# openai/Video-Pre-Training

Hardware: AMD Instinct MI355X
Metric: frames/sec (fwd) [+ bc_step.ms_per_step], 2x policy, 128x128x3 seq=128 (higher is better)
Workload: dtype bf16; 1 GPU; foundation-model-2x policy forward (IMPALA CNN + 4-layer banded transformer + heads), batch=64 seq=128 uint8 128x128x3 frames per GPU, KV memory carried, random-init weights; global_batch=64, seq_len=128, parallelism=dp1 replicas (no collective in forward; BC step: gradient all-reduce)

## Files before the change

### include/vpt_hip.h

```cpp
#ifndef VPT_HIP_H
#define VPT_HIP_H
#include <stdint.h>

#ifdef __cplusplus
extern "C" {
#endif

const char* vpt_version(void);
#define VPT_HIP_ABI 5
int vpt_abi_version(void);
const char* vpt_operand_format(void);
const char* vpt_last_error(void);

long vpt_conv3x3_packed_elems(int Cout, int Cin);
long vpt_conv3x3_table_floats(int Cout);
long vpt_linear_packed_elems(int N, int K);
long vpt_conv_first_packed_elems(int Cout);
long vpt_conv3d_t5_packed_elems(int O);
int vpt_pack_conv_first(const float* weight, const float* bias, void* wfrag, int Cout, void* stream);
int vpt_pack_conv3d_t5(const float* weight, const float* bias, void* wfrag, float* bias_padded, int O, void* stream);
int vpt_chw_to_blocked(const float* src, float* dst, int64_t rows, int C, int H, int W, void* stream);

enum { VPT_WS_CONV3X3_WGRAD = 1, VPT_WS_CONV_BACKWARD_PREPARE = 2, VPT_WS_LINEAR_SPLITK = 3, VPT_WS_LAYERNORM_BACKWARD = 4, VPT_WS_COLUMN_SUM = 5,
       VPT_WS_ATTENTION_BACKWARD_DKV = 6, VPT_WS_ATTENTION_BACKWARD_DBND = 7, VPT_WS_FRAME_AFFINE_BACKWARD = 8, VPT_WS_CONV_FIRST_BACKWARD = 9,
// ... 47 lines not shown

int vpt_linear_forward(const void* A, const void* wpk, const float* bias, const float* res,
                       float* out_f32, void* out_bf16, int M, int N, int K,
                       int lda, int ldr, int ldc, int ldcb, int relu, int splitk, const void* mask, int ldm,
                       void* stream);
int vpt_linear_forward_tiled(const void* A, const void* wpk, const float* bias, const float* res,
                             float* out_f32, void* out_bf16, int M, int N, int K,
                             int lda, int ldr, int ldc, int ldcb, int relu, int splitk, const void* mask, int ldm,
                             int tiling, void* stream);

int vpt_linear_wgrad(const void* dy, const void* x, float* dw, int M, int N, int K, int ldy, int ldx, int ldw, int accumulate, void* stream);

int vpt_dense_fold_epilogue(const float* part, int splitk, const double* stats, int count, const float* sg, const float* sb, float* out,
                            int M, int N, void* stream);

int vpt_linear_splitk_epilogue(const float* part, int splitk, const float* bias, const float* res, float* out_f32, void* out_bf16,
                               int M, int N, int ldr, int ldc, int ldcb, int relu, const void* mask, int ldm, void* stream);

int vpt_layernorm_linear_forward(const float* x, const float* ln_gain, const float* ln_bias, int relu_in, float* ln_out_f32,
                                 const void* wpk, const float* bias, const float* res, float* out_f32, void* out_bf16,
                                 int M, int N, int K, int ldr, int ldc, int ldcb, int relu, void* stream);

int vpt_layernorm_forward(const float* x, const float* gain, const float* bias, float* out_f32, void* out_bf16,
                          int M, int D, int relu_in, void* stream);

int vpt_masked_attention_forward(const float* qkvr, const float* kmem, const float* vmem, const uint8_t* memvalid,
                                 const float* b_nd, void* out, int B, int t, int heads, int hid, int ld,
                                 int maxlen, int causal, void* stream);

int vpt_masked_attention_forward_episodes(const float* qkvr, const float* kmem, const float* vmem, const uint8_t* memvalid,
                                          const float* b_nd, void* out, const int32_t* qlo, int B, int t, int heads, int hid, int ld,
                                          int maxlen, void* stream);

int vpt_episode_bounds(const uint8_t* first, const uint8_t* state_mask, int32_t* qlo, uint8_t* mask_out, int B, int t, int maxlen, void* stream);

int vpt_kv_memory_update(const float* qkvr, const float* kmem, const float* vmem, float* kout, float* vout,
                         int B, int t, int hid, int ld, int maxlen, void* stream);

int vpt_masked_attention_step(const float* qkvr, const float* kmem, const float* vmem, const uint8_t* state_mask, const uint8_t* first,
                              const float* b_nd, void* out, float* kout, float* vout, uint8_t* mask_out,
                              int B, int heads, int hid, int ld, int maxlen, void* stream);

int vpt_masked_attention_step_inplace(const float* qkvr, float* kmem, float* vmem, uint8_t* state_mask, const uint8_t* first,
                                      const float* b_nd, void* out, int* done_counter, int B, int heads, int hid, int ld, int maxlen, void* stream);

int vpt_act_epilogue(const int64_t* action_buttons, const int64_t* action_camera, const float* logp_buttons, const float* logp_camera,
                     const float* logits, int ld, int value_col, float scale, float shift, int64_t* keep, uint8_t* nan_flag, uint64_t* rng_state,
                     int B, void* stream);

int vpt_log_softmax_forward(const float* logits, float* out, int M, int ld, int col0, int n, float temperature,
                            void* stream);

int vpt_action_head_forward(const float* logits, const uint8_t* mask, const float* noise, const uint64_t* rng_state, uint32_t rng_stream,
                            float* out, int64_t* action, float* action_logp, int M, int ld, int col0, int n, float temperature, void* stream);
int vpt_uniform_noise(const uint64_t* rng_state, uint32_t rng_stream, float* out, int M, int n, void* stream);

int vpt_adam_step(float* param, const float* grad, float* exp_avg, float* exp_avg_sq, uint64_t n, int step,
                  float lr, float beta1, float beta2, float eps, float weight_decay, float grad_scale, void* stream);

int vpt_adam_step_multi(const void* table, int ntensors, int64_t total_blocks, int step, float lr, float beta1, float beta2,
                        float eps, float weight_decay, float grad_scale, const int32_t* skip_flag, void* stream);

int vpt_grads_nonfinite_multi(const void* table, int ntensors, int64_t total_blocks, int32_t* flag, void* stream);

long vpt_grad_norm_workspace_bytes(int ntensors, int64_t total_blocks);
int vpt_grad_norm_multi(const void* table, int ntensors, int64_t total_blocks, float grad_scale, float max_norm, void* workspace,
// ... 133 lines not shown
```

### video-pre-training_amd/_native.py

```python
import ctypes
import os

_HERE = os.path.dirname(os.path.abspath(__file__))
_LIB_PATH = os.environ.get("VPT_HIP_LIB") or os.path.join(_HERE, "libvpt_hip.so")
_LIB_PATHS = {"bf16": _LIB_PATH, "fp16": os.path.join(_HERE, "libvpt_hip_f16.so")}
_libs = {}

ABI_VERSION = 5

_P = ctypes.c_void_p
_I = ctypes.c_int
_F = ctypes.c_float
_L = ctypes.c_long
_D = ctypes.c_double

SIGNATURES = {
    "vpt_conv_first_forward": [_P, _P, _P, _P, _P, _P, _I, _I, _I, _I, _P],
    "vpt_conv3d_t5_forward": [_P, _P, _P, _P, _P, _I, _I, _I, _I, _I, _P],
    "vpt_conv3d_t5_forward_indexed": [_P, _P, _P, _P, _P, _P, _P, _P, _I, _I, _I, _I, _I, _P],
    "vpt_conv3d_t5_backward": [_P, _P, _P, _P, _P, _P, _I, _I, _I, _I, _I, _P],
    "vpt_gather_rows": [_P, _P, _P, _L, _L, _I, _P],
    "vpt_idm_decode": [_P] * 9 + [_L, _I, _D, _D, _D, _I, _P],
    "vpt_pack_conv3x3": [_P, _P, _P, _P, _P, _P, _I, _I, _P],
    "vpt_pack_linear": [_P, _P, _I, _I, _I, _I, _I, _P],
# ... 37 lines not shown
    "vpt_frame_affine_backward": [_P, _P, _P, _P, _P, _P, _P, _P, _P, _P, _I, _I, _I, _I, _I, _P],
    "vpt_bc_nll_backward": [_P, _P, _P, _P, _P, _I, _I, _I, _I, _F, _P],
    "vpt_bc_loss": [_P, _P, _P, _P, _P, _P, _P, _P, _P, _I, _I, _I, _I, _F, _P],
    "vpt_idm_loss": [_P, _P, _P, _P, _P, _P, _P, _P, _P, _I, _I, _I, _I, _I, _I, _F, _P],
    "vpt_rl_loss": [_P] * 9 + [ctypes.c_int64] + [_P] * 7 + [_I, _I, _I, _I, _F, _F, _F, _F, _F, _F, _P],
    "vpt_ppg_aux_loss": [_P] * 5 + [ctypes.c_int64] + [_P] * 7 + [_I, _I, _I, _I, _F, _F, _F, _F, _P],
    "vpt_gae": [_P, _P, _P, _P, _P, _P, _P, _I, _I, _F, _F, _P],
    "vpt_rollout_record": [_P] * 6 + [ctypes.c_int64] * 4 + [_P] * 7 + [_I, _I, _I, ctypes.c_int64, _P],
    "vpt_rollout_reward": [_P] * 7 + [_I, _I, _I, _P],
    "vpt_full_attention_backward": [_P, _P, _P, _P, _I, _I, _I, _I, _I, _P],
    "vpt_heads_logprob_backward": [_P, _P, _P, _P, _P, _P, _P, _P, _I, _I, _I, _I, _F, _F, _P],
    "vpt_grouped_logprob_backward": [_P, _P, _P, _P, _P, _P, _P, _I, _I, _I, _I, _I, _I, _F, _F, _P],
    "vpt_layernorm_backward": [_P, _P, _P, _P, _P, _P, _P, _P, _I, _I, _I, _P],
    "vpt_gate_cast": [_P, _P, _P, _I, _I, _I, _I, _I, _P],
    "vpt_column_sum": [_P, _P, _P, _I, _I, _I, _P],
    "vpt_masked_attention_backward": [_P, _P, _P, _P, _P, _P, _P, _P, _P, _P, _I, _I, _I, _I, _I, _I, _P],
    "vpt_adam_step": [_P, _P, _P, _P, ctypes.c_uint64, _I, _F, _F, _F, _F, _F, _F, _P],
    "vpt_adam_step_multi": [_P, _I, _L, _I, _F, _F, _F, _F, _F, _F, _P, _P],
    "vpt_grads_nonfinite_multi": [_P, _I, _L, _P, _P],
    "vpt_grad_norm_workspace_bytes": [_I, ctypes.c_int64],
    "vpt_grad_norm_multi": [_P, _I, _L, _F, _F, _P, _P, _P, _P, _P],
    "vpt_adam_step_multi_clip": [_P, _I, _L, _I, _F, _F, _F, _F, _F, _F, _P, _P, _P],
    "vpt_grad_accumulate_multi": [_P, _I, _L, _P],
    "vpt_layernorm_linear_forward": [_P, _P, _P, _I, _P, _P, _P, _P, _P, _P, _I, _I, _I, _I, _I, _I, _I, _P],
    "vpt_masked_attention_step": [_P, _P, _P, _P, _P, _P, _P, _P, _P, _P, _I, _I, _I, _I, _I, _P],
    "vpt_masked_attention_step_inplace": [_P, _P, _P, _P, _P, _P, _P, _P, _I, _I, _I, _I, _I, _P],
    "vpt_act_epilogue": [_P, _P, _P, _P, _P, _I, _I, _F, _F, _P, _P, _P, _I, _P],
    "vpt_clip_frames": [_P, _I, _I, _I, _P, _P, _P, _I, _I, _P, _I, _I, _P],
    "vpt_augment_uniforms": [_P, _P, _L, ctypes.c_uint64, ctypes.c_uint32, _P],
    "vpt_augment_frames": [_P, _P, _P, _L, _I, _I, _P],
    "vpt_debug_poison_lds": [_P],
    "vpt_episode_bounds": [_P, _P, _P, _P, _I, _I, _I, _P],
    "vpt_masked_attention_forward_episodes": [_P, _P, _P, _P, _P, _P, _P, _I, _I, _I, _I, _I, _I, _P],
    "vpt_masked_attention_backward_episodes": [_P, _P, _P, _P, _P, _P, _P, _P, _P, _P, _P, _I, _I, _I, _I, _I, _I, _P],
}


class NativeLibraryError(RuntimeError):
    pass


def lib_path():
    return _LIB_PATH


def load(fmt: str = "bf16"):
    if fmt in _libs:
        return _libs[fmt]
    import torch
    path = _LIB_PATHS[fmt]
    if not os.path.exists(path):
        raise NativeLibraryError(
            f"{path} is missing: run `python __graft_entry__.py` (build()) first; there is no CPU fallback")
    lib = ctypes.CDLL(path)
    try:
        lib.vpt_abi_version.restype = ctypes.c_int
        abi = int(lib.vpt_abi_version())
    except AttributeError:
        abi = None
    if abi != ABI_VERSION:
        raise NativeLibraryError(f"{path} has C-ABI version {abi}, this package binds version {ABI_VERSION}: rebuild it (`python __graft_entry__.py`)")
    override = fmt == "bf16" and bool(os.environ.get("VPT_HIP_LIB"))
    for name, argtypes in SIGNATURES.items():
        try:
            fn = getattr(lib, name)
        except AttributeError:
# ... 32 lines not shown
```

### video-pre-training_amd/csrc/vpt_capi.hip

```cpp
#include "../../include/vpt_hip.h"
#include "vpt_kernels.h"
#include "vpt_common.h"
#include <stdio.h>
#include <math.h>

static thread_local char g_err[256] = "ok";

static int fail(int code, const char* what) {
  snprintf(g_err, sizeof(g_err), "%s (code %d, hip: %s)", what, code, hipGetErrorString(hipPeekAtLastError()));
  return code;
}
#define CHECK_LAUNCH(expr, name) do { int rc_ = (expr); if (rc_ != 0) return fail(rc_, name); return 0; } while (0)

__global__ __launch_bounds__(256) void vpt_poison_lds_kernel(int words, unsigned pattern) {
  extern __shared__ unsigned poison_lds_[];
  volatile unsigned* l = poison_lds_;
  for (int i = threadIdx.x; i < words; i += 256) l[i] = pattern;
  __syncthreads();
  for (int k = 0; k < 16; ++k) __builtin_amdgcn_s_sleep(127);
}

extern "C" {

const char* vpt_version(void) { return "vpt_hip 0.5 gfx950"; }
// ... 393 lines not shown
  a.A = nullptr; a.wpk = nullptr; a.bias = bias; a.res = res; a.out_f32 = out_f32; a.out_bf16 = (vpt_op16*)out_bf16;
  a.M = M; a.N = N; a.K = 0; a.lda = 0; a.ldr = ldr; a.ldc = ldc; a.ldcb = ldcb; a.relu = relu; a.splitk = splitk; a.atomic_out = 0;
  a.mask = (const vpt_op16*)mask; a.ldm = ldm;
  CHECK_LAUNCH(vpt_splitk_epilogue_launch(part, splitk, &a, (hipStream_t)stream), "vpt_linear_splitk_epilogue");
}

int vpt_layernorm_forward(const float* x, const float* gain, const float* bias, float* out_f32, void* out_bf16,
                          int M, int D, int relu_in, void* stream) {
  VptLayerNormArgs a = {};
  a.x = x; a.gain = gain; a.bias = bias; a.out_f32 = out_f32; a.out_bf16 = (vpt_op16*)out_bf16;
  a.M = M; a.D = D; a.relu_in = relu_in;
  CHECK_LAUNCH(vpt_layernorm_launch(&a, (hipStream_t)stream), "vpt_layernorm_forward");
}

int vpt_masked_attention_forward(const float* qkvr, const float* kmem, const float* vmem, const uint8_t* memvalid,
                                 const float* b_nd, void* out, int B, int t, int heads, int hid, int ld,
                                 int maxlen, int causal, void* stream) {
  VptAttnArgs a = {};
  a.qkvr = qkvr; a.kmem = kmem; a.vmem = vmem; a.memvalid = memvalid; a.b_nd = b_nd; a.out = (vpt_op16*)out;
  a.B = B; a.t = t; a.heads = heads; a.hid = hid; a.ld = ld; a.maxlen = maxlen; a.causal = causal;
  CHECK_LAUNCH(vpt_attn_launch(&a, (hipStream_t)stream), "vpt_masked_attention_forward");
}

int vpt_masked_attention_forward_episodes(const float* qkvr, const float* kmem, const float* vmem, const uint8_t* memvalid,
                                          const float* b_nd, void* out, const int32_t* qlo, int B, int t, int heads, int hid, int ld,
                                          int maxlen, void* stream) {
  if (!qlo) return fail(-1, "vpt_masked_attention_forward_episodes: qlo ([B*t] int32, vpt_episode_bounds) is required");
  VptAttnArgs a = {};
  a.qkvr = qkvr; a.kmem = kmem; a.vmem = vmem; a.memvalid = memvalid; a.b_nd = b_nd; a.out = (vpt_op16*)out; a.qlo = qlo;
  a.B = B; a.t = t; a.heads = heads; a.hid = hid; a.ld = ld; a.maxlen = maxlen; a.causal = 1;
  CHECK_LAUNCH(vpt_attn_launch(&a, (hipStream_t)stream), "vpt_masked_attention_forward_episodes");
}

int vpt_episode_bounds(const uint8_t* first, const uint8_t* state_mask, int32_t* qlo, uint8_t* mask_out, int B, int t, int maxlen, void* stream) {
  if (!first || B <= 0 || t < 1 || maxlen < 1) return fail(-1, "vpt_episode_bounds: first [B][t] with B, t, maxlen >= 1 is required");
  if (mask_out && !state_mask) return fail(-1, "vpt_episode_bounds: mask_out needs state_mask");
  if (mask_out && mask_out == state_mask) return fail(-1, "vpt_episode_bounds: mask_out must not alias state_mask");
  CHECK_LAUNCH(vpt_episode_bounds_launch(first, state_mask, qlo, mask_out, B, t, maxlen, (hipStream_t)stream), "vpt_episode_bounds");
}

int vpt_masked_attention_step(const float* qkvr, const float* kmem, const float* vmem, const uint8_t* state_mask, const uint8_t* first,
                              const float* b_nd, void* out, float* kout, float* vout, uint8_t* mask_out,
                              int B, int heads, int hid, int ld, int maxlen, void* stream) {
  VptAttnArgs a = {};
  a.qkvr = qkvr; a.kmem = kmem; a.vmem = vmem; a.memvalid = nullptr; a.b_nd = b_nd; a.out = (vpt_op16*)out;
  a.B = B; a.t = 1; a.heads = heads; a.hid = hid; a.ld = ld; a.maxlen = maxlen; a.causal = 1;
  CHECK_LAUNCH(vpt_attn_step_launch(&a, state_mask, first, mask_out, kout, vout, nullptr, (hipStream_t)stream), "vpt_masked_attention_step");
}

int vpt_masked_attention_step_inplace(const float* qkvr, float* kmem, float* vmem, uint8_t* state_mask, const uint8_t* first,
                                      const float* b_nd, void* out, int* done_counter, int B, int heads, int hid, int ld, int maxlen, void* stream) {
  if (!done_counter) return fail(-1, "vpt_masked_attention_step_inplace: done_counter ([B] ints, zero before the first launch) is required");
  VptAttnArgs a = {};
  a.qkvr = qkvr; a.kmem = kmem; a.vmem = vmem; a.memvalid = nullptr; a.b_nd = b_nd; a.out = (vpt_op16*)out;
  a.B = B; a.t = 1; a.heads = heads; a.hid = hid; a.ld = ld; a.maxlen = maxlen; a.causal = 1;
  CHECK_LAUNCH(vpt_attn_step_launch(&a, state_mask, first, state_mask, kmem, vmem, done_counter, (hipStream_t)stream), "vpt_masked_attention_step_inplace");
}

int vpt_act_epilogue(const int64_t* action_buttons, const int64_t* action_camera, const float* logp_buttons, const float* logp_camera,
                     const float* logits, int ld, int value_col, float scale, float shift, int64_t* keep, uint8_t* nan_flag, uint64_t* rng_state,
                     int B, void* stream) {
  CHECK_LAUNCH(vpt_act_epilogue_launch(action_buttons, action_camera, logp_buttons, logp_camera, logits, ld, value_col, scale, shift, keep, nan_flag,
                                       rng_state, B, (hipStream_t)stream), "vpt_act_epilogue");
}

int vpt_uniform_noise(const uint64_t* rng_state, uint32_t rng_stream, float* out, int M, int n, void* stream) {
// ... 355 lines not shown
```

### video-pre-training_amd/csrc/vpt_kernels.h

```cpp
#pragma once
#include <hip/hip_runtime.h>
#include <stdint.h>

#ifdef VPT_OPERAND_F16
typedef _Float16 vpt_op16;
#else
typedef __bf16 vpt_op16;
#endif

struct VptConv3x3Args {
  const vpt_op16* x;
  const vpt_op16* wpk;
  const float* edge_sa;
  const float* edge_sg;
  const double* stats_in;
  const vpt_op16* res;
  vpt_op16* y;
  double* stats_out;
  int frames, H, W, Cin, Cout, CoutPad, NT;
  double inv_count_in;
  int tiling;
  int ablate;
  long long* trace;
  const float* kk_frame;
// ... 124 lines not shown
  int ldm;
  const float* ln_x;
  const float* ln_gain;
  const float* ln_bias;
  float* ln_out_f32;
  int ln_relu_in;
};

struct VptGemmTnArgs {
  const vpt_op16* A;
  const vpt_op16* B;
  float* C;
  int M, N1, N2, lda, ldb, ldc, accumulate;
};

struct VptLayerNormArgs {
  const float* x;
  const float* gain;
  const float* bias;
  float* out_f32;
  vpt_op16* out_bf16;
  int M, D, relu_in;
};

struct VptAttnArgs {
  const float* qkvr;
  const float* kmem;
  const float* vmem;
  const uint8_t* memvalid;
  const float* b_nd;
  vpt_op16* out;
  int B, t, heads, hid, ld, maxlen, causal;
  const int32_t* qlo;
};

struct VptKvUpdateArgs {
  const float* qkvr;
  const float* kmem;
  const float* vmem;
  float* kout;
  float* vout;
  int B, t, hid, ld, maxlen;
};

struct VptLogSoftmaxArgs {
  const float* logits;
  float* out;
  int M, ld, col0, n;
  float temperature;
  const uint8_t* mask;
  const float* noise;
  const uint64_t* rng_state;
  uint32_t rng_stream;
  long* action;
  float* action_logp;
};

struct VptAffineBwdArgs {
  const vpt_op16* x;
  const vpt_op16* dy;
  const vpt_op16* dx_add;
  vpt_op16* dx;
  const float* gain;
  const double* stats_in;
  double* ab;
  float* dgain;
// ... 373 lines not shown
```

### video-pre-training_amd/csrc/vpt_transformer.hip

```cpp
#include "vpt_common.h"
#include "vpt_kernels.h"

__global__ __launch_bounds__(256) void vpt_layernorm_kernel(VptLayerNormArgs a) {
  const int lane = threadIdx.x & 63;
  const int row = blockIdx.x * 4 + (threadIdx.x >> 6);
  if (row >= a.M) return;
  const float* x = a.x + (size_t)row * a.D;
  const int n4 = a.D >> 2;
  float s = 0.f;
  for (int i = lane; i < n4; i += 64) {
    f32x4 v = *(const f32x4*)(x + 4 * i);
    if (a.relu_in) { v.x = fmaxf(v.x, 0.f); v.y = fmaxf(v.y, 0.f); v.z = fmaxf(v.z, 0.f); v.w = fmaxf(v.w, 0.f); }
    s += (v.x + v.y) + (v.z + v.w);
  }
  const float mean = wave_sum(s) / (float)a.D;
  float ss = 0.f;
  for (int i = lane; i < n4; i += 64) {
    f32x4 v = *(const f32x4*)(x + 4 * i);
    if (a.relu_in) { v.x = fmaxf(v.x, 0.f); v.y = fmaxf(v.y, 0.f); v.z = fmaxf(v.z, 0.f); v.w = fmaxf(v.w, 0.f); }
    const float d0 = v.x - mean, d1 = v.y - mean, d2 = v.z - mean, d3 = v.w - mean;
    ss += (d0 * d0 + d1 * d1) + (d2 * d2 + d3 * d3);
  }
  const float rstd = rsqrtf(wave_sum(ss) / (float)a.D + VPT_NORM_EPS);
  for (int i = lane; i < n4; i += 64) {
// ... 31 lines not shown
#define ATT_QL_OFF (ATT_SC_OFF + ATT_QT)
#define ATT_PT_OFF ((ATT_QL_OFF + ATT_QT + 3) & ~3)
#define ATT_FLOATS (ATT_PT_OFF + 4 * 16 * 64)

__global__ __launch_bounds__(256) void vpt_attn_kernel(VptAttnArgs a) {
  extern __shared__ __attribute__((aligned(16))) float sm[];
  float* Ss = sm + ATT_S_OFF;
  float* Rs = sm + ATT_R_OFF;
  float* Bs = sm + ATT_B_OFF;
  float* Sc = sm + ATT_SC_OFF;
  int* Ql = (int*)(sm + ATT_QL_OFF);

  const int tid = threadIdx.x, lane = tid & 63, w = __builtin_amdgcn_readfirstlane(tid >> 6);
  const int b = blockIdx.y / a.heads, h = blockIdx.y - b * a.heads;
  const int q0 = blockIdx.x * ATT_QT;
  const int maxlen = a.maxlen, t = a.t, hid = a.hid;
  const size_t tok0 = (size_t)b * t;
  const int jbase = a.causal ? q0 + 1 : 0;

  for (int idx = tid; idx < ATT_QT * 10; idx += 256) {
    const int r = idx / 10, n = idx - r * 10;
    Rs[idx] = (a.causal && q0 + r < t) ? a.qkvr[(tok0 + q0 + r) * a.ld + 3 * hid + h * 10 + n] : 0.f;
  }
  for (int idx = tid; idx < 10 * maxlen; idx += 256) Bs[idx] = a.b_nd[idx];
  if (tid < ATT_QT) Ql[tid] = (a.qlo && q0 + tid < t) ? a.qlo[tok0 + q0 + tid] : 0;
  __syncthreads();

  const int l31 = lane & 31, hi = lane >> 5;
  auto kv_row = [&](int j, int which) -> const float* {
    if (j < maxlen) return (which == 1 ? a.kmem : a.vmem) + ((size_t)b * maxlen + j) * hid + h * ATT_DH;
    if (j - maxlen < t) return a.qkvr + (tok0 + j - maxlen) * a.ld + which * hid + h * ATT_DH;
    return nullptr;
  };
  {
    f32x16 acc, acc4;
#pragma unroll
    for (int r = 0; r < 16; ++r) { acc[r] = 0.f; acc4[r] = 0.f; }
    const f32x4 z4 = {0.f, 0.f, 0.f, 0.f};
    const float* qa = (q0 + l31 < t) ? a.qkvr + (tok0 + q0 + l31) * a.ld + h * ATT_DH + 4 * hi : nullptr;
    const float* kr = kv_row(jbase + w * 32 + l31, 1);
    const float* kr4 = kv_row(jbase + 128 + l31, 1);
    const float* kb = kr ? kr + 4 * hi : nullptr;
    const float* kb4 = kr4 ? kr4 + 4 * hi : nullptr;
#pragma unroll 8
    for (int g = 0; g < 16; ++g) {
      const f32x4 q4 = qa ? *(const f32x4*)(qa + 8 * g) : z4, k4 = kb ? *(const f32x4*)(kb + 8 * g) : z4;
      acc = __builtin_amdgcn_mfma_f32_32x32x2f32(q4.x, k4.x, acc, 0, 0, 0);
      acc = __builtin_amdgcn_mfma_f32_32x32x2f32(q4.y, k4.y, acc, 0, 0, 0);
      acc = __builtin_amdgcn_mfma_f32_32x32x2f32(q4.z, k4.z, acc, 0, 0, 0);
      acc = __builtin_amdgcn_mfma_f32_32x32x2f32(q4.w, k4.w, acc, 0, 0, 0);
    }
#pragma unroll
    for (int g4 = 0; g4 < 4; ++g4) {
      const int g = 4 * w + g4;
      const f32x4 q4 = qa ? *(const f32x4*)(qa + 8 * g) : z4, k4 = kb4 ? *(const f32x4*)(kb4 + 8 * g) : z4;
      acc4 = __builtin_amdgcn_mfma_f32_32x32x2f32(q4.x, k4.x, acc4, 0, 0, 0);
      acc4 = __builtin_amdgcn_mfma_f32_32x32x2f32(q4.y, k4.y, acc4, 0, 0, 0);
      acc4 = __builtin_amdgcn_mfma_f32_32x32x2f32(q4.z, k4.z, acc4, 0, 0, 0);
      acc4 = __builtin_amdgcn_mfma_f32_32x32x2f32(q4.w, k4.w, acc4, 0, 0, 0);
    }
    float* Pt = sm + ATT_PT_OFF;
#pragma unroll
    for (int r = 0; r < 16; ++r) Pt[(w * 16 + r) * 64 + lane] = acc4[r];
    __syncthreads();
    auto finish = [&](int kk, int r, float dot) {
      const int qi = (r & 3) + 8 * (r >> 2) + 4 * hi;
      const bool qvalid = (q0 + qi) < t;
      const int off = maxlen - 1 + qi - kk;
      const int j = jbase + kk;
      bool vis = a.causal ? (qvalid && off >= 0 && off < maxlen) : (qvalid && kk < t);
      if (vis && a.causal && j < maxlen) vis = a.memvalid[(size_t)b * maxlen + j] != 0;
      vis = vis && j >= Ql[qi];
      float sc = -3.0e38f;
      if (vis) {
        float rb = 0.f;
        if (a.causal) {
#pragma unroll
          for (int n = 0; n < 10; ++n) rb = fmaf(Rs[qi * 10 + n], Bs[n * maxlen + off], rb);
        }
        sc = dot * (1.0f / ATT_DH) + rb;
      }
      Ss[qi * ATT_SS + kk] = sc;
    };
#pragma unroll
    for (int r = 0; r < 16; ++r) finish(w * 32 + l31, r, acc[r]);
#pragma unroll
    for (int r4 = 0; r4 < 4; ++r4) {
      const int r = 4 * w + r4;
      const float dot = (Pt[(0 * 16 + r) * 64 + lane] + Pt[(1 * 16 + r) * 64 + lane]) + (Pt[(2 * 16 + r) * 64 + lane] + Pt[(3 * 16 + r) * 64 + lane]);
      finish(128 + l31, r, dot);
    }
  }
  __syncthreads();
  for (int r = w * 8; r < w * 8 + 8; ++r) {
    float* srow = Ss + r * ATT_SS;
    const float s0 = srow[lane], s1 = srow[lane + 64], s2 = (lane + 128 < ATT_NK) ? srow[lane + 128] : -3.0e38f;
    const float m = wave_max(fmaxf(s0, fmaxf(s1, s2)));
    const float e0 = (s0 > -1.0e38f) ? expf(s0 - m) : 0.f;
    const float e1 = (s1 > -1.0e38f) ? expf(s1 - m) : 0.f;
    const float e2 = (s2 > -1.0e38f) ? expf(s2 - m) : 0.f;
    const float tot = wave_sum(e0 + e1 + e2);
    srow[lane] = e0;
    srow[lane + 64] = e1;
    if (lane + 128 < ATT_NK) srow[lane + 128] = e2;
    if (lane == 0) Sc[r] = (tot > 0.f) ? 1.0f / tot : 0.f;
  }
  __syncthreads();

  {
    f32x16 o;
#pragma unroll
    for (int r = 0; r < 16; ++r) o[r] = 0.f;
    const float* pa = Ss + l31 * ATT_SS + 4 * hi;
    const int dcol = w * 32 + l31;
#pragma unroll 4
    for (int g = 0; g < ATT_NK / 8; ++g) {
      const f32x4 p4 = *(const f32x4*)(pa + 8 * g);
      float v[4];
#pragma unroll
      for (int e = 0; e < 4; ++e) {
        const float* r0 = kv_row(jbase + 8 * g + e, 2);
        const float* r1 = kv_row(jbase + 8 * g + 4 + e, 2);
        const float* rr = hi ? r1 : r0;
        v[e] = rr ? rr[dcol] : 0.f;
      }
      o = __builtin_amdgcn_mfma_f32_32x32x2f32(p4.x, v[0], o, 0, 0, 0);
      o = __builtin_amdgcn_mfma_f32_32x32x2f32(p4.y, v[1], o, 0, 0, 0);
      o = __builtin_amdgcn_mfma_f32_32x32x2f32(p4.z, v[2], o, 0, 0, 0);
      o = __builtin_amdgcn_mfma_f32_32x32x2f32(p4.w, v[3], o, 0, 0, 0);
    }
#pragma unroll
    for (int r = 0; r < 16; ++r) {
      const int qi = (r & 3) + 8 * (r >> 2) + 4 * hi;
      if (q0 + qi < t) a.out[(tok0 + q0 + qi) * hid + h * ATT_DH + w * 32 + l31] = (vpt_op16)(o[r] * Sc[qi]);
    }
  }
}

extern "C" int vpt_attn_launch(const VptAttnArgs* a, hipStream_t stream) {
  if (a->hid != a->heads * ATT_DH) return -1;
  if (a->causal ? (a->maxlen < 1 || a->maxlen > 129) : (a->maxlen != 0 || a->t > ATT_NK)) return -1;
  if (a->qlo && !a->causal) return -1;
  static unsigned long long optin_done = 0;
  const size_t lds = ATT_FLOATS * sizeof(float);
  if (!vpt_lds_optin((const void*)vpt_attn_kernel, (int)lds, &optin_done)) return -4;
  dim3 grid((a->t + ATT_QT - 1) / ATT_QT, a->B * a->heads);
  hipLaunchKernelGGL(vpt_attn_kernel, grid, dim3(256), lds, stream, *a);
  return hipGetLastError() == hipSuccess ? 0 : -3;
}

struct VptAttnStepExtra {
  const uint8_t* state_mask;
  const uint8_t* first;
  uint8_t* mask_out;
  float* kout;
  float* vout;
  int* done;
};

__global__ __launch_bounds__(256) void vpt_attn_step_kernel(VptAttnArgs a, VptAttnStepExtra x) {
  __shared__ float sc_[128], red_[8], part_[128];
  __shared__ int last_;
  const int tid = threadIdx.x, lane = tid & 63, w = tid >> 6;
  const int b = blockIdx.x / a.heads, h = blockIdx.x - b * a.heads;
  const int maxlen = a.maxlen, hid = a.hid;
  const float* qrow = a.qkvr + (size_t)b * a.ld;
  auto kv_row = [&](int j, int which) -> const float* {
    if (j < maxlen) return (which == 1 ? a.kmem : a.vmem) + ((size_t)b * maxlen + j) * hid + h * ATT_DH;
    return qrow + which * hid + h * ATT_DH;
  };
  const int kk = tid >> 1, half = tid & 1;
  const bool live = kk < maxlen;
  const int j = 1 + kk;
  f32x4 kv[16];
  float s = -3.0e38f;
// ... 275 lines not shown
```

### video-pre-training_amd/engine.py

```python
import contextlib
import os
from typing import Dict, List, Optional

import torch

from . import ops, packing

DENSE_SPLITK = int(os.environ.get("VPT_DENSE_SPLITK", "32"))


def config_from_policy_kwargs(policy_kwargs: dict, pi_head_kwargs: Optional[dict] = None) -> dict:
    pk = policy_kwargs
    width = pk.get("impala_width", 1)
    chans = [int(width * c) for c in pk.get("impala_chans", (16, 32, 32))]
    cfg = dict(
        chans=chans,
        hidsize=pk.get("hidsize", 512),
        heads=pk.get("attention_heads", 8),
        n_layers=pk.get("n_recurrence_layers", 1),
        maxlen=pk.get("attention_memory_size", 2048) - (pk.get("timesteps") or 0),
        causal=pk.get("attention_mask_style", "clipped_causal") == "clipped_causal",
        pointwise_ratio=pk.get("pointwise_ratio", 4),
        use_pre_lstm_ln=pk.get("use_pre_lstm_ln", True),
        temperature=float((pi_head_kwargs or {}).get("temperature", 1.0)),
# ... 466 lines not shown
        step = t == 1 and maxlen <= ops.ATTENTION_STEP_MAXLEN
        if inplace_state and not step:
            raise ValueError("inplace_state is the acting step's option (T = 1)")
        if step:
            first8 = first[:, 0].contiguous().view(torch.uint8)
        else:
            episodes = EpisodeMasks(first, bsz, t, maxlen, episode_starts)
        state_out = []
        for l in range(cfg["n_layers"]):
            state_mask, (kmem, vmem) = state_in[l]
            b_nd = w[f"net.recurrent_layer.blocks.{l}.b_nd"]
            if step:
                if state_mask is None:
                    state_mask = torch.zeros(bsz, 1, maxlen, dtype=torch.bool, device=x.device)
                done = None
                if inplace_state:
                    if not (kmem.is_contiguous() and vmem.is_contiguous()):
                        raise ValueError("inplace_state needs contiguous state tensors (a .contiguous() copy would receive the update instead of the state)")
                    if not state_mask.is_contiguous():
                        raise ValueError("inplace_state needs contiguous state masks")
                    if self._attn_done is None or self._attn_done.device != x.device:
                        self._attn_done = torch.zeros(64, dtype=torch.int32, device=x.device)
                    done = self._attn_done

                def attend(qkvr):
                    att, kout, vout, m8 = ops.masked_attention_step(qkvr, kmem.contiguous(), vmem.contiguous(), state_mask.reshape(bsz, maxlen).contiguous(), first8,
                                                                   b_nd, bsz, heads, hid, dtype=self.dtype, inplace=inplace_state, done=done)
                    state_out.append((state_mask if inplace_state else m8.view(torch.bool).view(bsz, 1, maxlen), (kout, vout)))
                    return att
            else:
                memvalid, new_mask = episodes.layer(state_mask, x.device)

                def attend(qkvr):
                    att = ops.masked_attention(qkvr, kmem.contiguous(), vmem.contiguous(), memvalid, b_nd, bsz, t, heads, hid, dtype=self.dtype, qlo=episodes.qlo)
                    state_out.append((new_mask, ops.kv_memory_update(qkvr, kmem.contiguous(), vmem.contiguous(), bsz, t, hid)))
                    return att
            x = self._block(x, l, tiling, 1, attend)

        _, y, _ = self._ln_linear(x, w["last.g"], w["last.b"], w["last.w"], hid, relu=True, relu_in=True, tiling=tiling)
        nb, nc = self.n_buttons, self.n_camera
        latent, logits, _ = self._ln_linear(y, w["final.g"], w["final.b"], w["heads.w"], nb + nc + 1, bias=w["heads.b"], ln_out_f32=True, tiling=tiling)
        temp = cfg["temperature"]
        out = dict(latent=latent.view(bsz, t, hid), state_out=state_out)
        tail = act_tail is not None and sample is not None and t == 1
        rng = self.rng_state(x.device) if sample == "stochastic" else None
        heads_out = action_heads(logits, (("buttons", 0, 1, nb), ("camera", nb, 1, nc)), bsz, t, temp, mask, sample, keep_head_logps=tail, rng_state=rng)
        out.update(heads_out)
        if tail:
            lps = out.pop("_head_logps")
            keep, flag = ops.act_epilogue(out["action"]["buttons"].view(-1), out["action"]["camera"].view(-1), lps["buttons"].reshape(-1),
                                          lps["camera"].reshape(-1), logits, nb + nc, act_tail[0], act_tail[1], rng_state=rng)
            out["_keep"], out["nan_flag"] = keep, flag
            out.update(unpack_act_tail(keep, bsz))
        else:
            out["vpred"] = logits[:, nb + nc:nb + nc + 1].reshape(bsz, t, 1).clone()
            if rng is not None:
                rng[1:].add_(1)
        return out


class IDMEngine(PolicyEngine):

    _QKV = "qkv"

    def __init__(self, cfg: dict, button_shape, camera_shape, cnn_chunk: int = 128, precision: Optional[str] = None):
        check_supported(cfg, idm=True)
        self._init_common(cfg, precision, cnn_chunk=cnn_chunk, cnn_streams=1, pool_subchunk=0, fuse_pool_sub=0)
        self.button_shape, self.camera_shape = tuple(button_shape), tuple(camera_shape)
# ... 118 lines not shown
```

### video-pre-training_amd/ops.py

```python
import ctypes
import os

import torch

from . import _native
from ._native import ptr


def _stream():
    return ctypes.c_void_p(torch.cuda.current_stream().cuda_stream)


class KernelTimer:

    def __init__(self):
        self.enabled = False
        self.records = []

    def reset(self):
        self.records = []

    def _accumulate(self, key_of):
        torch.cuda.synchronize()
        out = {}
# ... 497 lines not shown


def _chk_qlo(qlo, batch, t):
    _chk(qlo, torch.int32, "qlo")
    if qlo.numel() != batch * t:
        raise ValueError(f"qlo must hold one int32 per frame ([{batch}, {t}]), got {tuple(qlo.shape)}")


def episode_bounds(first, state_mask, maxlen, want_qlo=True, want_mask=True):
    if first.dtype == torch.bool:
        first = first.view(torch.uint8)
    _chk(first, torch.uint8, "first")
    if first.dim() != 2 or first.shape[1] < 1:
        raise ValueError(f"episode_bounds: first must be [batch, t >= 1], got {tuple(first.shape)}")
    batch, t = first.shape
    qlo = mout = None
    if want_mask:
        if state_mask is None:
            raise ValueError("episode_bounds: the next mask needs state_mask")
        if state_mask.dtype == torch.bool:
            state_mask = state_mask.view(torch.uint8)
        _chk(state_mask, torch.uint8, "state_mask")
        if tuple(state_mask.shape) != (batch, maxlen):
            raise ValueError(f"episode_bounds: state_mask must be [{batch}, {maxlen}], got {tuple(state_mask.shape)}")
        mout = torch.empty_like(state_mask)
    if want_qlo:
        qlo = torch.empty(batch, t, dtype=torch.int32, device=first.device)
    if batch and (want_qlo or want_mask):
        _call("vpt_episode_bounds", dict(bytes=5.0 * batch * t + 2.0 * batch * maxlen), ptr(first), ptr(state_mask) if want_mask else None, ptr(qlo), ptr(mout),
              batch, t, int(maxlen), _stream())
    return qlo, mout


def masked_attention(qkvr, kmem, vmem, memvalid, b_nd, batch, t, heads, hid, dtype=torch.bfloat16, qlo=None):
    _chk(qkvr, torch.float32, "qkvr"); _chk(kmem, torch.float32, "kmem"); _chk(vmem, torch.float32, "vmem")
    _chk(memvalid, torch.uint8, "memvalid"); _chk(b_nd, torch.float32, "b_nd")
    maxlen = kmem.shape[1]
    dt, fmt = _fmt(dtype=dtype)
    out = torch.empty(batch * t, hid, dtype=dt, device=qkvr.device)
    if qlo is not None:
        _chk_qlo(qlo, batch, t)
        _call("vpt_masked_attention_forward_episodes", dict(flops=4.0 * batch * t * (t + maxlen) * hid), ptr(qkvr), ptr(kmem), ptr(vmem), ptr(memvalid), ptr(b_nd),
              ptr(out), ptr(qlo), batch, t, heads, hid, qkvr.shape[1], maxlen, _stream(), fmt=fmt)
        return out
    _call("vpt_masked_attention_forward", dict(flops=4.0 * batch * t * (t + maxlen) * hid), ptr(qkvr), ptr(kmem), ptr(vmem), ptr(memvalid), ptr(b_nd), ptr(out),
                 batch, t, heads, hid, qkvr.shape[1], maxlen, 1, _stream(), fmt=fmt)
    return out


def kv_memory_update(qkvr, kmem, vmem, batch, t, hid):
    _chk(qkvr, torch.float32, "qkvr"); _chk(kmem, torch.float32, "kmem"); _chk(vmem, torch.float32, "vmem")
    kout, vout = torch.empty_like(kmem), torch.empty_like(vmem)
    _call("vpt_kv_memory_update", dict(bytes=16.0 * batch * kmem.shape[1] * hid), ptr(qkvr), ptr(kmem), ptr(vmem), ptr(kout), ptr(vout),
                 batch, t, hid, qkvr.shape[1], kmem.shape[1], _stream())
    return kout, vout


ATTENTION_STEP_MAXLEN = 128


def masked_attention_step(qkvr, kmem, vmem, state_mask, first, b_nd, batch, heads, hid, dtype=torch.bfloat16, inplace=False, done=None):
    _chk(qkvr, torch.float32, "qkvr"); _chk(kmem, torch.float32, "kmem"); _chk(vmem, torch.float32, "vmem"); _chk(b_nd, torch.float32, "b_nd")
    if state_mask.dtype == torch.bool:
        state_mask = state_mask.view(torch.uint8)
    if first.dtype == torch.bool:
        first = first.view(torch.uint8)
    _chk(state_mask, torch.uint8, "state_mask"); _chk(first, torch.uint8, "first")
    maxlen = kmem.shape[1]
    if qkvr.shape[0] != batch or maxlen > ATTENTION_STEP_MAXLEN or tuple(state_mask.shape) != (batch, maxlen) or first.numel() != batch:
        raise ValueError(f"masked_attention_step: one token per sequence, maxlen <= {ATTENTION_STEP_MAXLEN}, state_mask [batch, maxlen], first [batch] "
                         f"(got {qkvr.shape[0]} rows for batch {batch}, maxlen {maxlen}, mask {tuple(state_mask.shape)})")
    dt, fmt = _fmt(dtype=dtype)
    out = torch.empty(batch, hid, dtype=dt, device=qkvr.device)
    meta = dict(flops=4.0 * batch * maxlen * hid, bytes=16.0 * batch * maxlen * hid)
# ... 728 lines not shown
```

### video-pre-training_amd/training.py

```python
import contextlib
import os
from typing import List, Optional

import torch
import torch.distributed as dist

from . import distributed as D
from . import ops
from .cnn_training import _tap_sum, conv_param_grads
from .engine import DENSE_SPLITK, EpisodeMasks, check_episode_starts
from .trainer_base import TrainerBase, _round_up, linear_backward


class BCTrainer(TrainerBase):
    def __init__(self, policy, lr: float = 0.000181, weight_decay: float = 0.039428, betas=(0.9, 0.999), eps: float = 1e-8,
                 train_cnn: bool = True, optimizer_state: bool = True, loss_scale: Optional[float] = None,
                 scale_growth_interval: int = 200, episode_starts: str = "chunk", max_grad_norm: Optional[float] = None):
        self._init_trainer(policy, lr, weight_decay, betas, eps, train_cnn, optimizer_state, loss_scale, scale_growth_interval, max_grad_norm)
        self.episode_starts = check_episode_starts(episode_starts)
        self.autograd_lift, self.autograd_overflows = 256.0, 0
        self.cnn_streams = int(os.environ.get("VPT_BC_STREAMS", self.engine.cnn_streams))
        self.force_exchange = os.environ.get("VPT_DP_FORCE_EXCHANGE", "0") == "1"
        self._arenas = None
        self._streams: List[torch.cuda.Stream] = []
# ... 61 lines not shown
        eng = self.engine
        self.policy._ensure_packed()
        cfg, w = eng.cfg, eng.w
        bsz, t = img_u8.shape[:2]
        m = bsz * t
        hid, heads = cfg["hidsize"], cfg["heads"]
        dev, dt = img_u8.device, self.dtype
        nb, nc = eng.n_buttons, eng.n_camera
        frames = img_u8.reshape(m, *img_u8.shape[2:]).contiguous()

        outs, cnn_saved = [], []
        streams, main = self._chunk_streams((m + eng.cnn_chunk - 1) // eng.cnn_chunk)
        for ci, i in enumerate(range(0, m, eng.cnn_chunk)):
            with (torch.cuda.stream(streams[ci % len(streams)]) if streams else contextlib.nullcontext()):
                if self.train_cnn:
                    xn, sv = self._cnn_forward_saving(frames[i:i + eng.cnn_chunk])
                    cnn_saved.append(sv)
                else:
                    xn = eng._cnn_chunk(frames[i:i + eng.cnn_chunk])
                d32, _ = ops.linear(xn.view(xn.shape[0], -1), w["net.img_process.cnn.dense.w"], 256, splitk=DENSE_SPLITK)
                outs.append(d32)
                del xn
        for st in streams:
            main.wait_stream(st)
        d = outs[0] if len(outs) == 1 else torch.cat(outs, 0)
        episodes = EpisodeMasks(first, bsz, t, cfg["maxlen"], self.episode_starts)
        qlo = episodes.qlo
        state_out = []

        def attend(l, p, qkvr):
            state_mask, (kmem, vmem) = state_in[l]
            memvalid, new_mask = episodes.layer(state_mask, dev)
            kmem, vmem = kmem.contiguous(), vmem.contiguous()
            att = ops.masked_attention(qkvr, kmem, vmem, memvalid, w[p + "b_nd"], bsz, t, heads, hid, dtype=dt, qlo=qlo)
            kout, vout = ops.kv_memory_update(qkvr, kmem, vmem, bsz, t, hid)
            state_out.append((new_mask, (kout, vout)))
            return att, dict(kmem=kmem, vmem=vmem, memvalid=memvalid, qlo=qlo)

        trunk = self._trunk_forward_saving(d, attend)
        x_trunk = trunk["x_trunk"]
        _, xb = ops.layernorm(x_trunk, w["last.g"], w["last.b"], relu_in=True, dtype=dt)
        y, y16 = ops.linear(xb, w["last.w"], hid, relu=True, out_f32=True, out_bf16=True)
        _, lb = ops.layernorm(y, w["final.g"], w["final.b"], dtype=dt)
        logits, _ = ops.linear(lb, w["heads.w"], nb + nc + 1, bias=w["heads.b"])
        temp = cfg["temperature"]
        mk = {h: (mask[h].reshape(m, n_).to(torch.uint8).contiguous() if mask is not None and mask.get(h) is not None else None)
              for h, n_ in (("buttons", nb), ("camera", nc))}
        lp_b = ops.log_softmax_cols(logits, 0, nb, temp, mask=mk["buttons"])
        lp_c = ops.log_softmax_cols(logits, nb, nc, temp, mask=mk["camera"])
        return dict(trunk, m=m, bsz=bsz, t=t, dev=dev, d=d, xb=xb, y=y, y16=y16, lb=lb, logits=logits, lp_b=lp_b, lp_c=lp_c,
                    cnn_saved=cnn_saved, state_out=state_out, ldz=_round_up(nb + nc + 1, 64), mask=mk)

    def _attention_backward(self, S, l, datt, g):
        cfg = self.engine.cfg
        p = f"net.recurrent_layer.blocks.{l}."
        s = S["saved"][l]
        db_nd = g[p + "r.orc_block.b_nd"] = torch.zeros(10, cfg["maxlen"], dtype=torch.float32, device=S["dev"])
        return ops.masked_attention_backward(s["qkvr"], s["kmem"], s["vmem"], s["memvalid"], self.engine.w[p + "b_nd"], datt,
                                             db_nd, S["bsz"], S["t"], cfg["heads"], cfg["hidsize"], qlo=s["qlo"])

    @torch.no_grad()
    def backward_from(self, S: dict, dz: torch.Tensor, on_trunk_grads=None, debug: Optional[dict] = None, value_grads: bool = False):
        eng = self.engine
        P = {n: p.detach() for n, p in self.params.items()}
        g, dd = self._trunk_backward(S, dz, P, value_grads=value_grads, debug=debug)
        if on_trunk_grads is not None:
            on_trunk_grads(g)
        if self.train_cnn:
# ... 204 lines not shown
```

Before: 79520 frames/s.

## Fuse KV memory update into masked attention forward kernel

The attention kernel now writes the updated K/V memory (kout/vout) itself, replacing the separate kv_memory_update launch in both the inference and training paths. Each block copies the slice of K/V rows it is responsible for. Some of those loads are issued early and their stores are placed after the score computation to hide latency. The V-operand loads for the PV MFMA are also hoisted into a register array ahead of the barrier. This saves one kernel launch and a second read of qkvr/kmem per layer, at the cost of higher register pressure in the attention kernel.

Result: no change. 79790 frames/s (median of 6 runs) (+0.3%).

```diff
diff --git a/include/vpt_hip.h b/include/vpt_hip.h
--- a/include/vpt_hip.h
+++ b/include/vpt_hip.h
@@ -103,6 +103,10 @@
                                           const float* b_nd, void* out, const int32_t* qlo, int B, int t, int heads, int hid, int ld,
                                           int maxlen, void* stream);
 
+int vpt_masked_attention_forward_update(const float* qkvr, const float* kmem, const float* vmem, const uint8_t* memvalid,
+                                        const float* b_nd, void* out, const int32_t* qlo, float* kout, float* vout,
+                                        int B, int t, int heads, int hid, int ld, int maxlen, void* stream);
+
 int vpt_episode_bounds(const uint8_t* first, const uint8_t* state_mask, int32_t* qlo, uint8_t* mask_out, int B, int t, int maxlen, void* stream);
 
 int vpt_kv_memory_update(const float* qkvr, const float* kmem, const float* vmem, float* kout, float* vout,
diff --git a/video-pre-training_amd/_native.py b/video-pre-training_amd/_native.py
--- a/video-pre-training_amd/_native.py
+++ b/video-pre-training_amd/_native.py
@@ -93,6 +93,7 @@
     "vpt_debug_poison_lds": [_P],
     "vpt_episode_bounds": [_P, _P, _P, _P, _I, _I, _I, _P],
     "vpt_masked_attention_forward_episodes": [_P, _P, _P, _P, _P, _P, _P, _I, _I, _I, _I, _I, _I, _P],
+    "vpt_masked_attention_forward_update": [_P, _P, _P, _P, _P, _P, _P, _P, _P, _I, _I, _I, _I, _I, _I, _P],
     "vpt_masked_attention_backward_episodes": [_P, _P, _P, _P, _P, _P, _P, _P, _P, _P, _P, _I, _I, _I, _I, _I, _I, _P],
 }
 
diff --git a/video-pre-training_amd/csrc/vpt_capi.hip b/video-pre-training_amd/csrc/vpt_capi.hip
--- a/video-pre-training_amd/csrc/vpt_capi.hip
+++ b/video-pre-training_amd/csrc/vpt_capi.hip
@@ -449,6 +449,18 @@
   CHECK_LAUNCH(vpt_attn_launch(&a, (hipStream_t)stream), "vpt_masked_attention_forward_episodes");
 }
 
+int vpt_masked_attention_forward_update(const float* qkvr, const float* kmem, const float* vmem, const uint8_t* memvalid,
+                                        const float* b_nd, void* out, const int32_t* qlo, float* kout, float* vout,
+                                        int B, int t, int heads, int hid, int ld, int maxlen, void* stream) {
+  if (!kout || !vout) return fail(-1, "vpt_masked_attention_forward_update: kout and vout ([B][maxlen][hid] fp32) are required");
+  VptAttnArgs a = {};
+  a.qkvr = qkvr; a.kmem = kmem; a.vmem = vmem; a.memvalid = memvalid; a.b_nd = b_nd; a.out = (vpt_op16*)out; a.qlo = qlo;
+  a.B = B; a.t = t; a.heads = heads; a.hid = hid; a.ld = ld; a.maxlen = maxlen; a.causal = 1; a.kout = kout; a.vout = vout;
+  const int rc = vpt_attn_launch(&a, (hipStream_t)stream);
+  if (rc == -5) return fail(rc, "vpt_masked_attention_forward_update: kout / vout must not overlap kmem / vmem or each other");
+  CHECK_LAUNCH(rc, "vpt_masked_attention_forward_update");
+}
+
 int vpt_episode_bounds(const uint8_t* first, const uint8_t* state_mask, int32_t* qlo, uint8_t* mask_out, int B, int t, int maxlen, void* stream) {
   if (!first || B <= 0 || t < 1 || maxlen < 1) return fail(-1, "vpt_episode_bounds: first [B][t] with B, t, maxlen >= 1 is required");
   if (mask_out && !state_mask) return fail(-1, "vpt_episode_bounds: mask_out needs state_mask");
diff --git a/video-pre-training_amd/csrc/vpt_kernels.h b/video-pre-training_amd/csrc/vpt_kernels.h
--- a/video-pre-training_amd/csrc/vpt_kernels.h
+++ b/video-pre-training_amd/csrc/vpt_kernels.h
@@ -180,6 +180,8 @@
   vpt_op16* out;
   int B, t, heads, hid, ld, maxlen, causal;
   const int32_t* qlo;
+  float* kout;
+  float* vout;
 };
 
 struct VptKvUpdateArgs {
diff --git a/video-pre-training_amd/csrc/vpt_transformer.hip b/video-pre-training_amd/csrc/vpt_transformer.hip
--- a/video-pre-training_amd/csrc/vpt_transformer.hip
+++ b/video-pre-training_amd/csrc/vpt_transformer.hip
@@ -87,6 +87,21 @@
     if (j - maxlen < t) return a.qkvr + (tok0 + j - maxlen) * a.ld + which * hid + h * ATT_DH;
     return nullptr;
   };
+  const int cr = tid >> 5, cc = 4 * (tid & 31);
+  const int cp_lo = a.kout ? max(q0 == 0 ? 1 : q0 + 129, t) : 0, cp_hi = a.kout ? min(q0 + 161, t + maxlen) : 0;
+  f32x4 ck[4], cv[4];
+#pragma unroll
+  for (int i = 0; i < 4; ++i) {
+    const int j = cp_lo + cr + 8 * i;
+    if (j < cp_hi) { ck[i] = *(const f32x4*)(kv_row(j, 1) + cc); cv[i] = *(const f32x4*)(kv_row(j, 2) + cc); }
+  }
+  for (int j = cp_lo + 32 + cr; j < cp_hi; j += 8) {
+    const size_t o = ((size_t)b * maxlen + (j - t)) * hid + h * ATT_DH + cc;
+    *(f32x4*)(a.kout + o) = *(const f32x4*)(kv_row(j, 1) + cc);
+    *(f32x4*)(a.vout + o) = *(const f32x4*)(kv_row(j, 2) + cc);
+  }
+  float v[ATT_NK / 8][4];
+  const int dcol = w * 32 + l31;
   {
     f32x16 acc, acc4;
 #pragma unroll
@@ -117,6 +132,25 @@
     float* Pt = sm + ATT_PT_OFF;
 #pragma unroll
     for (int r = 0; r < 16; ++r) Pt[(w * 16 + r) * 64 + lane] = acc4[r];
+#pragma unroll
+    for (int g = 0; g < ATT_NK / 8; ++g) {
+#pragma unroll
+      for (int e = 0; e < 4; ++e) {
+        const float* r0 = kv_row(jbase + 8 * g + e, 2);
+        const float* r1 = kv_row(jbase + 8 * g + 4 + e, 2);
+        const float* rr = hi ? r1 : r0;
+        v[g][e] = rr ? rr[dcol] : 0.f;
+      }
+    }
+#pragma unroll
+    for (int i = 0; i < 4; ++i) {
+      const int j = cp_lo + cr + 8 * i;
+      if (j < cp_hi) {
+        const size_t o = ((size_t)b * maxlen + (j - t)) * hid + h * ATT_DH + cc;
+        *(f32x4*)(a.kout + o) = ck[i];
+        *(f32x4*)(a.vout + o) = cv[i];
+      }
+    }
     __syncthreads();
     auto finish = [&](int kk, int r, float dot) {
       const int qi = (r & 3) + 8 * (r >> 2) + 4 * hi;
@@ -167,22 +201,13 @@
 #pragma unroll
     for (int r = 0; r < 16; ++r) o[r] = 0.f;
     const float* pa = Ss + l31 * ATT_SS + 4 * hi;
-    const int dcol = w * 32 + l31;
-#pragma unroll 4
+#pragma unroll
     for (int g = 0; g < ATT_NK / 8; ++g) {
       const f32x4 p4 = *(const f32x4*)(pa + 8 * g);
-      float v[4];
-#pragma unroll
-      for (int e = 0; e < 4; ++e) {
-        const float* r0 = kv_row(jbase + 8 * g + e, 2);
-        const float* r1 = kv_row(jbase + 8 * g + 4 + e, 2);
-        const float* rr = hi ? r1 : r0;
-        v[e] = rr ? rr[dcol] : 0.f;
-      }
-      o = __builtin_amdgcn_mfma_f32_32x32x2f32(p4.x, v[0], o, 0, 0, 0);
-      o = __builtin_amdgcn_mfma_f32_32x32x2f32(p4.y, v[1], o, 0, 0, 0);
-      o = __builtin_amdgcn_mfma_f32_32x32x2f32(p4.z, v[2], o, 0, 0, 0);
-      o = __builtin_amdgcn_mfma_f32_32x32x2f32(p4.w, v[3], o, 0, 0, 0);
+      o = __builtin_amdgcn_mfma_f32_32x32x2f32(p4.x, v[g][0], o, 0, 0, 0);
+      o = __builtin_amdgcn_mfma_f32_32x32x2f32(p4.y, v[g][1], o, 0, 0, 0);
+      o = __builtin_amdgcn_mfma_f32_32x32x2f32(p4.z, v[g][2], o, 0, 0, 0);
+      o = __builtin_amdgcn_mfma_f32_32x32x2f32(p4.w, v[g][3], o, 0, 0, 0);
     }
 #pragma unroll
     for (int r = 0; r < 16; ++r) {
@@ -190,12 +215,24 @@
       if (q0 + qi < t) a.out[(tok0 + q0 + qi) * hid + h * ATT_DH + w * 32 + l31] = (vpt_op16)(o[r] * Sc[qi]);
     }
   }
+}
+
+static bool vpt_ranges_overlap(const float* p, const float* q, size_t n) {
+  const uintptr_t p0 = (uintptr_t)p, q0 = (uintptr_t)q, bytes = n * sizeof(float);
+  return p0 < q0 + bytes && q0 < p0 + bytes;
 }
 
 extern "C" int vpt_attn_launch(const VptAttnArgs* a, hipStream_t stream) {
   if (a->hid != a->heads * ATT_DH) return -1;
   if (a->causal ? (a->maxlen < 1 || a->maxlen > 129) : (a->maxlen != 0 || a->t > ATT_NK)) return -1;
   if (a->qlo && !a->causal) return -1;
+  if ((a->kout != nullptr) != (a->vout != nullptr) || (a->kout && !a->causal)) return -1;
+  if (a->kout) {
+    const size_t n = (size_t)a->B * a->maxlen * a->hid;
+    if (vpt_ranges_overlap(a->kout, a->kmem, n) || vpt_ranges_overlap(a->kout, a->vmem, n) || vpt_ranges_overlap(a->vout, a->kmem, n) ||
+        vpt_ranges_overlap(a->vout, a->vmem, n) || vpt_ranges_overlap(a->kout, a->vout, n))
+      return -5;
+  }
   static unsigned long long optin_done = 0;
   const size_t lds = ATT_FLOATS * sizeof(float);
   if (!vpt_lds_optin((const void*)vpt_attn_kernel, (int)lds, &optin_done)) return -4;
diff --git a/video-pre-training_amd/engine.py b/video-pre-training_amd/engine.py
--- a/video-pre-training_amd/engine.py
+++ b/video-pre-training_amd/engine.py
@@ -522,8 +522,10 @@
                 memvalid, new_mask = episodes.layer(state_mask, x.device)
 
                 def attend(qkvr):
-                    att = ops.masked_attention(qkvr, kmem.contiguous(), vmem.contiguous(), memvalid, b_nd, bsz, t, heads, hid, dtype=self.dtype, qlo=episodes.qlo)
-                    state_out.append((new_mask, ops.kv_memory_update(qkvr, kmem.contiguous(), vmem.contiguous(), bsz, t, hid)))
+                    km, vm = kmem.contiguous(), vmem.contiguous()
+                    kout, vout = torch.empty_like(km), torch.empty_like(vm)
+                    att = ops.masked_attention(qkvr, km, vm, memvalid, b_nd, bsz, t, heads, hid, dtype=self.dtype, qlo=episodes.qlo, kout=kout, vout=vout)
+                    state_out.append((new_mask, (kout, vout)))
                     return att
             x = self._block(x, l, tiling, 1, attend)
 
diff --git a/video-pre-training_amd/ops.py b/video-pre-training_amd/ops.py
--- a/video-pre-training_amd/ops.py
+++ b/video-pre-training_amd/ops.py
@@ -553,7 +553,7 @@
     return qlo, mout
 
 
-def masked_attention(qkvr, kmem, vmem, memvalid, b_nd, batch, t, heads, hid, dtype=torch.bfloat16, qlo=None):
+def masked_attention(qkvr, kmem, vmem, memvalid, b_nd, batch, t, heads, hid, dtype=torch.bfloat16, qlo=None, kout=None, vout=None):
     _chk(qkvr, torch.float32, "qkvr"); _chk(kmem, torch.float32, "kmem"); _chk(vmem, torch.float32, "vmem")
     _chk(memvalid, torch.uint8, "memvalid"); _chk(b_nd, torch.float32, "b_nd")
     maxlen = kmem.shape[1]
@@ -561,6 +561,17 @@
     out = torch.empty(batch * t, hid, dtype=dt, device=qkvr.device)
     if qlo is not None:
         _chk_qlo(qlo, batch, t)
+    if (kout is None) != (vout is None):
+        raise ValueError("masked_attention: give both kout and vout or neither")
+    if kout is not None:
+        _chk(kout, torch.float32, "kout"); _chk(vout, torch.float32, "vout")
+        if kout.shape != kmem.shape or vout.shape != vmem.shape:
+            raise ValueError(f"masked_attention: kout / vout must be shaped like kmem / vmem {tuple(kmem.shape)}, got {tuple(kout.shape)} / {tuple(vout.shape)}")
+        _call("vpt_masked_attention_forward_update", dict(flops=4.0 * batch * t * (t + maxlen) * hid, bytes=16.0 * batch * maxlen * hid), ptr(qkvr), ptr(kmem), ptr(vmem),
+              ptr(memvalid), ptr(b_nd), ptr(out), ptr(qlo), ptr(kout), ptr(vout), batch, t, heads, hid, qkvr.shape[1], maxlen, _stream(), fmt=fmt,
+              label="vpt_masked_attention_forward")
+        return out
+    if qlo is not None:
         _call("vpt_masked_attention_forward_episodes", dict(flops=4.0 * batch * t * (t + maxlen) * hid), ptr(qkvr), ptr(kmem), ptr(vmem), ptr(memvalid), ptr(b_nd),
               ptr(out), ptr(qlo), batch, t, heads, hid, qkvr.shape[1], maxlen, _stream(), fmt=fmt)
         return out
diff --git a/video-pre-training_amd/training.py b/video-pre-training_amd/training.py
--- a/video-pre-training_amd/training.py
+++ b/video-pre-training_amd/training.py
@@ -117,8 +117,8 @@
             state_mask, (kmem, vmem) = state_in[l]
             memvalid, new_mask = episodes.layer(state_mask, dev)
             kmem, vmem = kmem.contiguous(), vmem.contiguous()
-            att = ops.masked_attention(qkvr, kmem, vmem, memvalid, w[p + "b_nd"], bsz, t, heads, hid, dtype=dt, qlo=qlo)
-            kout, vout = ops.kv_memory_update(qkvr, kmem, vmem, bsz, t, hid)
+            kout, vout = torch.empty_like(kmem), torch.empty_like(vmem)
+            att = ops.masked_attention(qkvr, kmem, vmem, memvalid, w[p + "b_nd"], bsz, t, heads, hid, dtype=dt, qlo=qlo, kout=kout, vout=vout)
             state_out.append((new_mask, (kout, vout)))
             return att, dict(kmem=kmem, vmem=vmem, memvalid=memvalid, qlo=qlo)
 
```
